# austintheriot/ray-tracer-webgl

Hardware: AMD Instinct MI355X
Metric: Mray/s (ray segments/s) at 1920x1080 (higher is better)
Workload: dtype f32

## Files before the change

profiles/summarize.py:

```python
#!/usr/bin/env python3
import csv
import glob
import json
import os
import sys
from collections import defaultdict

if sys.argv[1] == "--merge":
    dst = os.path.join(os.path.dirname(os.path.abspath(__file__)), "pmc_traffic.json")
    doc = json.load(open(dst)) if os.path.exists(dst) else {}
    recs = doc.get("records") or ([doc] if doc.get("kernel") else [])
    for src in sys.argv[2:]:
        rec = json.load(open(os.path.join(src, "pmc_traffic.json")))
        recs = [r for r in recs if not (r.get("kernel") == rec.get("kernel") and str(r.get("config", "2")) == str(rec.get("config", "2")))]
        recs.append(rec)
        print("merged %s config %s from %s" % (rec.get("kernel"), rec.get("config"), src))
    recs.sort(key=lambda r: str(r.get("config", "2")))
    json.dump({"note": "one record per (kernel, config): the counter-derived figures bench.py attaches (labelled PRIOR) to a line of the "
                       "same kernel, config and launch shape; written by profiles/summarize.py from a profiles/collect.sh run",
               "records": recs}, open(dst, "w"), indent=1)
    sys.exit(0)
d = sys.argv[1]
out = {}
bench = {}
try:
    for line in open(os.path.join(d, "kt.log")):
        if line.startswith("{") and '"metric"' in line:
            bench = json.loads(line)
except Exception:
    bench = {}
cfg_name = (bench.get("config", {}).get("workload", "config2").split(":")[0] or "config2")
cfg_key = cfg_name.replace("config", "")
ppl = int(bench.get("config", {}).get("passes_per_launch", 64))
spp_pass = int(bench.get("config", {}).get("spp_per_pass", 16))
for f in glob.glob(os.path.join(d, "kt", "**", "*_kernel_stats.csv"), recursive=True):
    print("== kernel-trace stats (%s)" % os.path.relpath(f, d))
    for row in csv.DictReader(open(f)):
        if row["Name"].startswith("pt_"):
            print("  %-24s calls %s avg %.3f ms min %.3f max %.3f  (%s %%)" % (
                row["Name"], row["Calls"], float(row["AverageNs"]) / 1e6, float(row["MinNs"]) / 1e6,
                float(row["MaxNs"]) / 1e6, row["Percentage"]))
            out.setdefault("kernel_stats", {})[row["Name"]] = {
                "calls": int(row["Calls"]), "avg_ms": float(row["AverageNs"]) / 1e6}
for f in glob.glob(os.path.join(d, "kt", "**", "*_kernel_trace.csv"), recursive=True):
    rows = [r for r in csv.DictReader(open(f)) if r["Kernel_Name"].startswith("pt_trace")]
    by = defaultdict(list)
    for r in rows:
        by[r["Kernel_Name"]].append((int(r["End_Timestamp"]) - int(r["Start_Timestamp"])) / 1e6)
    print("== full-size dispatches per trace kernel (%s)" % os.path.relpath(f, d))
    for k, v in sorted(by.items()):
        full = [x for x in v if x >= 0.85 * max(v)]
        print("  %-32s %d of %d dispatches full-size: avg %.3f ms  min %.3f  max %.3f" % (k, len(full), len(v), sum(full) / len(full), min(full), max(full)))
        out.setdefault("kernel_full", {})[k] = {"calls": len(full), "avg_ms": sum(full) / len(full)}
for f in glob.glob(os.path.join(d, "kt_configs", "**", "*_kernel_trace.csv"), recursive=True):
    print("== trace-kernel dispatches of tools/config_sweep.py config3 config4 config5 default (%s)" % os.path.relpath(f, d))
    rows = [r for r in csv.DictReader(open(f)) if r["Kernel_Name"].startswith("pt_trace")]
    rows.sort(key=lambda r: int(r["Start_Timestamp"]))
    for r in rows:
        print("  %-32s %9.3f ms  grid %s threads in workgroups of %s  lds %s B  vgpr %s+%s sgpr %s" % (
            r["Kernel_Name"], (int(r["End_Timestamp"]) - int(r["Start_Timestamp"])) / 1e6, r.get("Grid_Size_X", "?"),
            r.get("Workgroup_Size_X", "?"), r.get("LDS_Block_Size", "?"), r.get("VGPR_Count", "?"),
            r.get("Accum_VGPR_Count", "?"), r.get("SGPR_Count", "?")))
for f in glob.glob(os.path.join(d, "kt_configs.log")):
    print("== tools/config_sweep.py output under the profiler")
    for line in open(f):
        if line.startswith(("config", "default")):
            print("  " + line.rstrip())
ctr = defaultdict(lambda: defaultdict(list))
seen_in = defaultdict(set)
for f in sorted(glob.glob(os.path.join(d, "pmc*", "**", "*_counter_collection.csv"), recursive=True)):
    rows = [r for r in csv.DictReader(open(f))]
    pass_dir = os.path.relpath(f, d).split(os.sep)[0]
    longest = defaultdict(float)
    for row in rows:
        dur = float(int(row["End_Timestamp"]) - int(row["Start_Timestamp"]))
        longest[row["Kernel_Name"]] = max(longest[row["Kernel_Name"]], dur)
    for row in rows:
        dur = float(int(row["End_Timestamp"]) - int(row["Start_Timestamp"]))
        if dur >= 0.85 * longest[row["Kernel_Name"]]:
            key = (row["Kernel_Name"], row["Counter_Name"])
            if seen_in[key] and pass_dir not in seen_in[key]:
                continue
            seen_in[key].add(pass_dir)
            ctr[row["Kernel_Name"]][row["Counter_Name"]].append((int(row["Dispatch_Id"]), float(row["Counter_Value"])))
main_kernel = None
if ctr:
    cands = [k for k in ctr if k.startswith("pt_trace")]
    main_kernel = max(cands, key=lambda k: max(len(v) for v in ctr[k].values())) if cands else None
for k in sorted(ctr):
    if not k.startswith("pt_trace"):
        continue
    print("== PMC per dispatch of %s (mean over dispatches; summed over XCDs/SEs by rocprofv3)%s" % (
        k, "  <-- timed kernel" if k == main_kernel else ""))
    vals = {}
    for name in sorted(ctr[k]):
        per = defaultdict(float)
        for disp, v in ctr[k][name]:
            per[disp] += v
        mean = sum(per.values()) / max(len(per), 1)
        vals[name] = mean
        print("  %-28s %.6g" % (name, mean))
    if k == main_kernel:
        out["pmc"] = vals
        out["pmc_kernel"] = k
    g = vals
    if "SQ_INSTS_VALU" in g and "GRBM_GUI_ACTIVE" in g:
        print("  -- derived: cycles per VALU instruction per SIMD = %.3f" % ((g["GRBM_GUI_ACTIVE"] / 8.0) * 1024.0 / g["SQ_INSTS_VALU"]))
    if "FETCH_SIZE" in g:
        print("  FETCH_SIZE KiB %.6g -> bytes %.6g (x2 if wide coalesced: %.6g)" % (g["FETCH_SIZE"], g["FETCH_SIZE"] * 1024, g["FETCH_SIZE"] * 2048))
    if "WRITE_SIZE" in g:
        print("  WRITE_SIZE KiB %.6g -> bytes %.6g" % (g["WRITE_SIZE"], g["WRITE_SIZE"] * 1024))
pm = out.get("pmc", {})
# ... 31 lines not shown
```

ray_tracer_webgl_amd/csrc/pt_api.hip:

```cpp
#include <hip/hip_runtime.h>

#include <mutex>
#include <chrono>
#include <cmath>
#include <cstdarg>
#include <cstdio>
#include <cstdlib>
#include <cstring>
#include <new>
#include <string>
#include <thread>
#include <utility>
#include <vector>

#include "../../include/ptrace.h"
#include "../../include/ptrace_dev.h"
#include "pt_bvh.hpp"
#include "pt_grid.hpp"
#include "pt_grid_records.hpp"
#include "pt_scene_image.hpp"
#include "pt_extra.h"
#include "pt_kernel_args.h"
#include "pt_geom_plan.hpp"
#include "pt_launch_plan.hpp"
// ... 981 lines not shown
    A.lds_scene_bytes = (uint32_t)scene;
  } else {
    const bool have_lds = c->list.n <= PT_MAX_SPHERES_LDS;
    scene = have_lds ? (size_t)PT_LDS_ENTRIES(c->list.n) * 16 : 0;
    row = path == PT_GEOM_SMALL ? ROW_SMALL + (int)(c->list.n & 3u)
                                : (path == PT_GEOM_LDS ? ROW_LIST_LDS : (have_lds ? ROW_SCALAR : ROW_SCALAR_NOLDS));
  }
  const int build = feat ? BUILD_FEAT : (dbg ? BUILD_DBG : (rr ? BUILD_RR : (c->count_work ? BUILD_TWIN : BUILD_PLAIN)));
  if (feat) {
    A.uuid = c->list.uuid.get();
    A.slot_uuid = path == PT_GEOM_BVH ? c->bvh.uuid.get() : (path == PT_GEOM_GRID ? c->grid.uuid.get() : nullptr);
    A.slab = reinterpret_cast<float*>(c->d_feat.get());
    A.spp = 1; A.max_depth = 1; A.rr_min_depth = 0;
  }
  if (walk && path == PT_GEOM_GRID && row == ROW_GRID && (build == BUILD_PLAIN || build == BUILD_TWIN)) {
    A.grid_cells = c->grid.ring.get();
    A.n_cells = (uint32_t)ptrec::ring_cells(c->grid.head.n[0], c->grid.head.n[2]);
  }
  const TraceKernel& tk = kTraceKernels[row][build];
  const void* kfn = tk.main ? tk.main
                            : (tk.feature >= 0 ? feature_kernel(c->device, tk.feature)
                            : tk.debug >= 0 ? debug_kernel(c->device, tk.debug)
                                             : (tk.extra >= 0 ? extra_kernel(c->device, tk.extra) : pt_small_kernel((unsigned)tk.small)));
  c->last_build = build;
  const uint32_t block = walk ? walk_block_threads(kfn, tk.waves, scene, kWalkLdsMax, knobs.bvh_block) : list_block_threads(scene);
  const size_t lds = walk ? scene + (size_t)PT_PARK_STRIDE * 4 * block : scene;
  A.block_threads = block;
  int per_cu = 0;
  PT_HIP(c, resident_blocks(kfn, block, lds, tk.waves, &per_cu));

  const LaunchPlan P = plan_launch({A.n_items, feat ? 1 : c->params.samples_per_pixel, n_passes, block, per_cu, (uint32_t)c->num_cus, walk,
                                    c->list.n, knobs});
  A.queue_chunk = P.queue_chunk; A.queue_static = (uint32_t)P.deal; A.queue_groups = P.queue_groups;
  A.n_waves = P.n_waves; A.coop_max_live = P.coop_max_live;
  A.cost_feedback = use.feedback == LaunchUse::PLANNED ? P.cost_feedback : (use.feedback == LaunchUse::ON ? 1u : 0u);
  if (feat) A.cost_feedback = 0u;
  L->kfn = kfn; L->grid = P.grid; L->block = block; L->lds = lds; L->path = path; L->trial = choice.trial;
  return PT_OK;
}

static int launch_trace(pt_ctx* c, const Launch& L) {
  void* kargs[] = {const_cast<PtKernelArgs*>(&L.A)};
  PT_HIP(c, hipLaunchKernel(L.kfn, dim3(L.grid), dim3(L.block), kargs, L.lds, c->stream));
  return PT_OK;
}

PT_API int pt_render_passes(pt_ctx* c, uint32_t n_passes) {
  if (!c) return PT_ERR_INVALID;
  if (!c->have_spheres || !c->have_params)
    return fail(c, PT_ERR_NOT_READY, "pt_render: pt_set_spheres and pt_set_params must come first");
  if (n_passes == 0) return fail(c, PT_ERR_INVALID, "pt_render_passes: n_passes == 0");
  if (n_passes > c->reserved_passes)
    return fail(c, PT_ERR_CAPACITY, "pt_render_passes: %u passes > %u reserved (pt_reserve_passes)",
                n_passes, c->reserved_passes);
  if (c->local_rows == 0) return PT_OK;
  const bool estimate = c->err_on && !c->err_paused;
  if (estimate && c->err_spp != 0 && c->err_spp != c->params.samples_per_pixel)
    return fail(c, PT_ERR_INVALID, "pt_render_passes: %d samples per pixel while the error estimate holds passes of %d: clear first "
                                   "(pt_reset_accum)", c->params.samples_per_pixel, c->err_spp);
  PT_HIP(c, hipSetDevice(c->device));

  Launch L;
  {
    LaunchUse use;
    use.allow_trials = true;
    int rc = prepare_launch(c, n_passes, use, &L);
    if (rc != PT_OK) return rc;
// ... 978 lines not shown
```

ray_tracer_webgl_amd/csrc/pt_kernel_args.h:

```cpp
#pragma once
#include <stdint.h>

struct PtMatRec {
  float albedo[3];
  float fuzz;
  float refraction_index;
  int32_t type;
  float radius;
  float inv_ri;
};
static_assert(sizeof(PtMatRec) == 32, "PtMatRec must be 32 bytes");
struct PtDiv {
  uint32_t m, s1, s2;
};
static inline PtDiv pt_div_make(uint32_t d) {
  PtDiv r;
  uint32_t l = 0;
  while (l < 32 && (1ull << l) < (unsigned long long)d) l++;
  r.m = (uint32_t)(((1ull << 32) * ((1ull << l) - d)) / d + 1ull);
  r.s1 = l < 1 ? l : 1;
  r.s2 = l > 0 ? l - 1 : 0;
  return r;
}

// ... 25 lines not shown
  const uint32_t* bvh_slot_index;
  const PtMatRec* slot_mat;
  uint32_t n_nodes, n_tree_slots, n_slots, n_outliers;
  float bvh_c0[3], bvh_s0;
  const uint32_t* grid_cells;
  uint32_t n_cells;
  uint32_t grid_n[3];
  float grid_lo[3], grid_hi[3], grid_h[3], grid_inv_h[3];
  float grid_r2_near;
  float grid_lo_n[3], grid_hi_n[3];
  uint32_t lds_scene_bytes;
  unsigned long long* wave_log;
  uint32_t refill_min;
  uint32_t carry_lanes;
  float bvh_kinv;
  uint32_t block_threads;
  uint32_t queue_chunk;
  float fw, fh;
  PtDiv div_per_tile, div_tiles_x, div_band_rows;
  uint32_t coop_max_live;
  int32_t rr_min_depth;
  uint32_t lens_off;
  uint32_t queue_groups;
  uint32_t queue_static;
  uint32_t n_waves;
  uint32_t cost_feedback;
  uint32_t* cell_hist;
  const uint32_t* frame_ctr;
  const float* mat_r0;
  const int32_t* uuid;
  const int32_t* slot_uuid;
  float dbg_cursor[3];
  int32_t dbg_selected;
};

#ifndef PT_WAVES_WALK
#define PT_WAVES_WALK 6
#endif
#ifndef PT_WAVES_LIST
#define PT_WAVES_LIST 7
#endif
#define PT_WAVES_LIST_LDS 6
#ifndef PT_WAVES_SMALL
#define PT_WAVES_SMALL 7
#endif
#define PT_WAVES_TWIN_CELLS 4
#define PT_BUILT_FOR(n) __attribute__((amdgpu_waves_per_eu(n, n)))
#ifndef PT_LEAF_GROUP_GMEM
#define PT_LEAF_GROUP_GMEM 4
#endif

enum { PT_WAVE_LOG_WORDS = 4 };
enum { PT_COH_BINS = 66, PT_HIST_WAVE_STRIDE = 8 };
enum { PT_REG_REFILL_DECODE = 0, PT_REG_REFILL_RESERVE, PT_REG_CAMERA_RAY, PT_REG_SHADE_HIT_RECORD, PT_REG_SHADE_SKY, PT_REG_SHADE_DIFFUSE,
       PT_REG_SHADE_METAL, PT_REG_SHADE_GLASS, PT_REG_SHADE_GLASS_REFRACT, PT_REG_SHADE_CONTINUES, PT_REG_SHADE_FINISHED, PT_REG_SHADE_ITEM_STORE,
       PT_REG_WALK_ENTRY, PT_REG_WALK_ENTER_CELL, PT_REG_WALK_FAR_RAY, PT_REG_SHADE_ANY, PT_N_REGIONS };
enum { PT_CTR_HEAD = 0, PT_CTR_SEGMENTS = 1, PT_CTR_SAMPLES = 2, PT_CTR_FAR_RAYS = 3 , PT_CTR_SCRATCH = 7 , PT_CTR_WORK = 8, PT_CTR_LITERAL = 16, PT_CTR_PHASES = 24, PT_N_PHASES = 8, PT_CTR_REGIONS = 32, PT_CTR_TIMEBINS = 64, PT_CTR_COUNT = 128,
       PT_QUEUE_GROUPS_MAX = 256, PT_CTR_GROUP_HEADS = 128 ,
       PT_CTR_ALLOC = PT_CTR_GROUP_HEADS + 8 * PT_QUEUE_GROUPS_MAX };

#define PT_LDS_ENTRIES(n) ((((n) + 7u) & ~7u) + 4u)
#define PT_MAX_SPHERES_SMALL 16u
#define PT_MAX_SPHERES_LDS 10232u
#define PT_PARK_DWORDS 14u
#ifndef PT_PARK_STRIDE
#define PT_PARK_STRIDE 15u
#endif
#define PT_BVH_LDS_BYTES32(n_nodes, n_slots) ((((size_t)(n_nodes) + 1u) * 2u + (size_t)(n_slots)) * 16u)
#define PT_BVH_LDS_BYTES16(n_nodes) (((size_t)(n_nodes) + 1u) * 16u)
#define PT_GRID_LDS_CELLS(n_cells) ((((size_t)(n_cells) + 3u) / 4u) * 16u)
#define PT_MAX_SPHERES 65528u

enum {
  PT_PROBE_HASH = 0,
  PT_PROBE_SINCOS = 1,
  PT_PROBE_CBRT = 2,
  PT_PROBE_UNIT_SPHERE = 3,
  PT_PROBE_DIVSQRT = 4,
  PT_PROBE_BASE_HASH = 5,
  PT_PROBE_FAST_ARITH = 6,
};
```

ray_tracer_webgl_amd/csrc/pt_launch_plan.hpp:

```cpp
#pragma once
#include <cstdint>
#include <optional>

#include "pt_kernel_args.h"

struct LaunchKnobs {
  std::optional<uint32_t> carry_lanes;
  std::optional<uint32_t> bvh_block;
  std::optional<uint32_t> coop_max;
  std::optional<int> per_cu;
  std::optional<uint32_t> queue_chunk;
  std::optional<uint32_t> grid_percent;
  std::optional<bool> queue_static;
  std::optional<bool> cost_feedback;
  std::optional<int> fewer_x10_1, fewer_x10_2;
  std::optional<bool> queue_grouped;
};

struct LaunchPlanIn {
  uint64_t items = 0;
  int spp = 1;
  uint32_t passes = 1;
  uint32_t block = 256;
  int per_cu = 1;
  uint32_t num_cus = 256;
  bool walk = false;
  uint32_t n_spheres = 0;
  LaunchKnobs knobs;
};

enum class Deal : uint32_t { Shared = 0, Static = 1, Grouped = 2 };

struct LaunchPlan {
  uint32_t queue_chunk = 0;
  Deal deal = Deal::Shared;
  uint32_t queue_groups = 0;
  uint32_t grid = 1;
  uint32_t n_waves = 0;
  uint32_t cost_feedback = 0;
  uint32_t coop_max_live = 0;
};

inline uint32_t list_block_threads(uint64_t lds) { return lds > 40 * 1024 ? 1024u : 256u; }

inline LaunchPlan plan_launch(const LaunchPlanIn& in) {
  const LaunchKnobs& k = in.knobs;
  const uint64_t items = in.items;
  const uint32_t block = in.block;
  LaunchPlan P;
  P.cost_feedback = (in.passes >= 2u || in.spp >= 8) ? 1u : 0u;
  if (!in.walk) {
    const uint32_t per_ray = (in.n_spheres / 64u + 1u) * 60u + 60u;
    const uint32_t lim = (12u * in.n_spheres + 700u) / per_ray;
    P.coop_max_live = lim > 16u ? 16u : lim;
    if (k.coop_max) P.coop_max_live = *k.coop_max;
  }
  int per_cu = in.per_cu < 1 ? 1 : in.per_cu;
  if (k.per_cu && *k.per_cu >= 1 && *k.per_cu <= 32) per_cu = *k.per_cu;

  {
    const unsigned long long lanes = (unsigned long long)in.num_cus * (unsigned)per_cu * block;
    P.queue_chunk = items >= 192ull * lanes ? 512u : (items >= 64ull * lanes ? 128u : (items >= 16ull * lanes ? 64u : 32u));
    {
      const uint32_t spp = (uint32_t)(in.spp > 0 ? in.spp : 1);
      uint32_t c_min = 32u;
      while (c_min * spp < 1100u && c_min < 1024u) c_min *= 2u;
      if (P.queue_chunk < c_min) P.queue_chunk = c_min;
    }
    if (k.queue_chunk && *k.queue_chunk >= 1u && *k.queue_chunk <= 4096u) P.queue_chunk = *k.queue_chunk;
  }
  const unsigned long long want = (items + block - 1) / block;
  const unsigned long long resident = (unsigned long long)in.num_cus * (unsigned)per_cu;
  uint32_t grid = (uint32_t)(want < resident ? want : resident);
  if (k.grid_percent) grid = (uint32_t)((unsigned long long)grid * *k.grid_percent / 100ull);
  if (grid < 1) grid = 1;
  P.grid = grid;
  P.n_waves = grid * (block / 64u);
  const unsigned long long lanes_all = (unsigned long long)P.n_waves * 64ull;
// ... 35 lines not shown
```

ray_tracer_webgl_amd/csrc/pt_refill.hpp:

```cpp
#pragma once
#include "pt_scene.hpp"

namespace ptk {

struct PixelDiv {
  bool wh_ok;
  float y_fw, y_fh;
};
__device__ __forceinline__ PixelDiv pixel_div() {
  karg_t& K = *kargs();
  PixelDiv pd;
  pd.wh_ok = div_den_ok(K.fw) && div_den_ok(K.fh);
  pd.y_fw = u2f((uint32_t)__builtin_amdgcn_readfirstlane((int)f2u(rcp_newton(K.fw))));
  pd.y_fh = u2f((uint32_t)__builtin_amdgcn_readfirstlane((int)f2u(rcp_newton(K.fh))));
  return pd;
}

template <bool FEAT = false>
__device__ __forceinline__ void start_sample(Path& p, const PixelDiv& pd) {
  karg_t& K = *kargs();
  if constexpr (FEAT) {
    const float s = p.st_s, t = p.st_t;
    const V3 dd = mk(fma_(t, K.vertical[0], fma_(s, K.horizontal[0], K.llc[0])),
                     fma_(t, K.vertical[1], fma_(s, K.horizontal[1], K.llc[1])),
// ... 22 lines not shown
  const V3 tt = mk(dd.x - cam_o.x, dd.y - cam_o.y, dd.z - cam_o.z);
  float seed_l = seed;
  seed = (seed + 0.1f) + 0.1f;
  seed = (seed + 0.1f) + 0.1f;
  bool lens = K.lens_off == 0u;
  if (!lens) {
    const uint32_t nz = 0x80000000u;
    lens = pt_ballot(f2u(tt.x) == nz || f2u(tt.y) == nz || f2u(tt.z) == nz) != 0ull;
  }
  if (lens) {
    float ua = hash1(seed_l);
    float sa, ca;
    sincos2pi(ua, sa, ca);
    float rr = sqrt_rn(hash1(seed_l));
    float rdx = K.lens_radius * (rr * ca);
    float rdy = K.lens_radius * (rr * sa);
    V3 off = mk(fma_(K.cam_v[0], rdy, K.cam_u[0] * rdx), fma_(K.cam_v[1], rdy, K.cam_u[1] * rdx),
                fma_(K.cam_v[2], rdy, K.cam_u[2] * rdx));
    d = mk(tt.x - off.x, tt.y - off.y, tt.z - off.z);
    o = mk(cam_o.x + off.x, cam_o.y + off.y, cam_o.z + off.z);
  } else {
    d = tt;
    o = cam_o;
  }
  a = dot3(d, d);
  col = mk(1.0f, 1.0f, 1.0f);
  depth = 0;
  p.seed = seed; p.o = o; p.d = d; p.a = a; p.col = col; p.depth = depth;
}

template <bool COUNT>
__device__ __forceinline__ void refill(const PtKernelArgs& A, Path& p, Queue& q, const PixelDiv& pd, Tally<COUNT>& tally) {
  karg_t& K = *kargs();
  bool alive = p.alive, new_path = p.new_path;
  bool dry = q.dry;
  uint32_t slab_index = p.slab_index, item_tile = p.item_tile, item_segs = p.item_segs;
  int sample = p.sample; float seed = p.seed, st_s = p.st_s, st_t = p.st_t; V3 sum = p.sum;
  uint32_t pool_next = q.pool_next, pool_end = q.pool_end, refill_waited = q.refill_waited;
  uint32_t pool_tp0 = q.pool_tp0, pool_split = q.pool_split, pool_tile0 = q.pool_tile0, pool_tile1 = q.pool_tile1;
  uint32_t q_round = q.round;
  const bool wh_ok = pd.wh_ok;
  const float y_fw = pd.y_fw, y_fh = pd.y_fh;
  bool dealt = false, put_off = false;
  for (;;) {
    bool need = !alive && !dry;
    unsigned long long mask = pt_ballot(need);
    if (mask == 0ull) break;
    if ((uint32_t)__popcll(mask) < K.refill_min && (uint32_t)__popcll(pt_ballot(alive)) >= 32u &&
        (dealt ? 0u : refill_waited) < 8u) {
      put_off = true;
      break;
    }
    dealt = true;
    if (pool_next == pool_end) {
      tally.flag(PT_REG_REFILL_RESERVE);
      unsigned long long base = 0;
      if (K.queue_static == 2u) {
        const uint32_t wave = blockIdx.x * (blockDim.x >> 6) + (threadIdx.x >> 6);
        const uint32_t group = wave & (K.queue_groups - 1u);
        unsigned long long r = 0;
        if (lane_id() == 0u) r = atomicAdd(&A.counters[PT_CTR_GROUP_HEADS + 8u * group], 1ull);
        const uint32_t r_lo = (uint32_t)__builtin_amdgcn_readfirstlane((int)(uint32_t)r);
        base = ((unsigned long long)r_lo * K.queue_groups + group) * (unsigned long long)A.queue_chunk;
      } else if (K.queue_static != 0u) {
        const uint32_t wave = blockIdx.x * (blockDim.x >> 6) + (threadIdx.x >> 6);
        base = ((unsigned long long)q_round * K.n_waves + wave) * (unsigned long long)A.queue_chunk;
        q_round++;
      } else {
        if (lane_id() == 0u) base = atomicAdd(&A.counters[PT_CTR_HEAD], (unsigned long long)A.queue_chunk);
      }
      base = ((unsigned long long)(uint32_t)__builtin_amdgcn_readfirstlane((int)(uint32_t)(base >> 32)) << 32) |
             (unsigned long long)(uint32_t)__builtin_amdgcn_readfirstlane((int)(uint32_t)base);
      if (base >= (unsigned long long)A.n_items) {
        tally.queue_dry();
        dry = true;
        need = false;
      } else {
        pool_next = (uint32_t)base;
        unsigned long long end = base + A.queue_chunk;
        pool_end = end < (unsigned long long)A.n_items ? (uint32_t)end : A.n_items;
        pool_tp0 = div_by(pool_next, K.div_per_tile.m, K.div_per_tile.s1, K.div_per_tile.s2);
        pool_split = (pool_tp0 + 1u) * (64u * K.n_passes);
        const uint32_t n_tiles_w = K.tiles_x * K.tiles_y;
        pool_tile0 = (uint32_t)__builtin_amdgcn_readfirstlane((int)K.tile_order[pool_tp0]);
        pool_tile1 = (uint32_t)__builtin_amdgcn_readfirstlane((int)K.tile_order[pool_tp0 + 1u < n_tiles_w ? pool_tp0 + 1u : pool_tp0]);
      }
    }
    const uint32_t avail = pool_end - pool_next;
    const uint32_t cnt = (uint32_t)__popcll(mask);
    const uint32_t rank = (uint32_t)__popcll(mask & ((1ull << lane_id()) - 1ull));
    const uint32_t pool_base = pool_next;
    pool_next += cnt < avail ? cnt : avail;
    if (need && rank < avail) {
      tally.flag(PT_REG_REFILL_DECODE);
      uint32_t item = pool_base + rank;
      uint32_t per_tile = 64u * K.n_passes;
      uint32_t tile_pos, tile;
      if (K.queue_chunk <= per_tile) {
        const bool second = item >= pool_split;
        tile_pos = pool_tp0 + (second ? 1u : 0u);
        const uint32_t t0 = pool_tile0, t1 = pool_tile1;
        tile = second ? t1 : t0;
      } else {
        tile_pos = div_by(item, K.div_per_tile.m, K.div_per_tile.s1, K.div_per_tile.s2);
        tile = K.tile_order[tile_pos];
      }
      uint32_t rem_i = item - tile_pos * per_tile;
      uint32_t pass = rem_i >> 6, l = rem_i & 63u;
      uint32_t ty = div_by(tile, K.div_tiles_x.m, K.div_tiles_x.s1, K.div_tiles_x.s2), tx = tile - ty * K.tiles_x;
      uint32_t px = tx * 8u + (l & 7u), ly = ty * 8u + (l >> 3);
      if (px < K.width && ly < K.local_rows) {
        uint32_t y = ly;
        if (K.band_count > 1u) {
          uint32_t b = div_by(ly, K.div_band_rows.m, K.div_band_rows.s1, K.div_band_rows.s2), r = ly - b * K.band_rows;
          y = (b * K.band_count + K.band_index) * K.band_rows + r;
        }
        const float fx2 = (float)(2u * px + 1u), fy2 = (float)(2u * y + 1u);
        float vx, vy;
        if (wh_ok) { vx = div_core(fx2, K.fw, y_fw) - 1.0f; vy = div_core(fy2, K.fh, y_fh) - 1.0f; }
        else { vx = fx2 / K.fw - 1.0f; vy = fy2 / K.fh - 1.0f; }
        const uint32_t frame_k = *(const uint32_t __attribute__((address_space(4)))*)K.frame_ctr;
        float u_time = K.time0 + (float)(K.first_pass + pass + frame_k) * K.time_step;
        seed = (float)base_hash(f2u(vx), f2u(vy)) * (1.0f / 4294967296.0f) + u_time;
        st_s = (vx + 1.0f) * 0.5f;
        st_t = (vy + 1.0f) * 0.5f;
        slab_index = (pass * K.local_rows + ly) * K.width + px;
        item_tile = (pass == 0u && K.cost_feedback != 0u) ? tile : 0xffffffffu;
        item_segs = 0;
        sum = mk(0.f, 0.f, 0.f);
        sample = 0;
        new_path = true;
        alive = true;
      }
    }
  }
  refill_waited = (dealt ? 0u : refill_waited) + (put_off ? 1u : 0u);
  p.alive = alive; p.new_path = new_path;
  p.slab_index = slab_index; p.item_tile = item_tile; p.item_segs = item_segs;
  p.sample = sample; p.seed = seed; p.st_s = st_s; p.st_t = st_t; p.sum = sum;
  q.pool_next = pool_next; q.pool_end = pool_end; q.refill_waited = refill_waited;
  q.pool_tp0 = pool_tp0; q.pool_split = pool_split; q.pool_tile0 = pool_tile0; q.pool_tile1 = pool_tile1;
  q.round = q_round; q.dry = dry;
}

}
```

ray_tracer_webgl_amd/csrc/pt_scene.hpp:

```cpp
#pragma once
#include "pt_arith.hpp"
#include "pt_kernel_args.h"

namespace ptk {
using namespace ptd;

extern __shared__ float4 pt_lds[];

typedef float f4v __attribute__((ext_vector_type(4)));
typedef const f4v __attribute__((address_space(4))) const_f4v;
typedef const PtKernelArgs __attribute__((address_space(4))) karg_t;

__device__ __forceinline__ karg_t* kargs() { return (karg_t*)__builtin_amdgcn_kernarg_segment_ptr(); }

__device__ __forceinline__ uint32_t lane_id() { return threadIdx.x & 63u; }

__device__ __forceinline__ uint32_t div_by(uint32_t n, uint32_t m, uint32_t s1, uint32_t s2) {
  const uint32_t t = __umulhi(m, n);
  return (t + ((n - t) >> s1)) >> s2;
}

struct Path {
  bool alive = false;
  bool new_path = false;
  uint32_t slab_index = 0;
  uint32_t item_tile = 0xffffffffu, item_segs = 0;
  int sample = 0, depth = 0;
  float seed = 0.f, st_s = 0.f, st_t = 0.f;
  V3 o = mk(0, 0, 0), d = mk(0, 0, 0);
  float a = 0.f;
  V3 col = mk(1, 1, 1), sum = mk(0, 0, 0);
};

struct Queue {
  uint32_t pool_next = 0, pool_end = 0;
  uint32_t refill_waited = 0;
  uint32_t pool_tp0 = 0, pool_split = 0, pool_tile0 = 0, pool_tile1 = 0;
  uint32_t round = 0;
  bool dry = false;
};

struct Hit {
  float closest = PT_MAX_T;
  int hit = -1;
  uint32_t lit_from = 0xffffffffu;
};

struct Carry {
  bool carried = false;
  float closest_w = PT_MAX_T;
  uint32_t hit_pos = 0xffffffffu;
};
struct BvhWalk {
  uint32_t cur = 0, l0 = 0, l1 = 0, l2 = 0, l3 = 0, l_cnt = 0;
  uint32_t q0 = 0, q1 = 0, q2 = 0, q3 = 0, q_cnt = 0;
};
struct GridWalk {
  float tmx = 0.f, tmy = 0.f, tmz = 0.f, t_exit = 0.f;
  uint32_t cell = 0, rem = 0, pend = 0;
};

template <bool SCAN_LDS_, bool HAVE_LDS_, int WALK_, int TAIL_ = -1, bool FLAT_Y_ = false>
struct Scene {
  static constexpr bool SCAN_LDS = SCAN_LDS_, HAVE_LDS = HAVE_LDS_;
  static constexpr int WALK = WALK_;
  static constexpr bool BVH = WALK >= 1 && WALK <= 3;
  static constexpr bool GRID = WALK >= 4 && WALK <= 6;
  static constexpr bool FLAT_Y = FLAT_Y_;
  static_assert(!FLAT_Y_ || WALK_ == 4, "the one-layer walk exists for the LDS-staged grid build");
// ... 169 lines not shown
  __device__ __forceinline__ void carried(bool c) { if constexpr (COUNT) n_carried += (uint32_t)__popcll(pt_ballot(c)); }
  __device__ __forceinline__ void literal(const PtKernelArgs& A, bool irregular, bool handed_over, uint32_t slab_index) {
    if constexpr (COUNT) {
      const unsigned long long mi = pt_ballot(irregular), mh = pt_ballot(handed_over);
      if ((mi | mh) != 0ull && lane_id() == 0) {
        atomicAdd(&A.counters[PT_CTR_LITERAL + 0], (unsigned long long)__popcll(mi));
        atomicAdd(&A.counters[PT_CTR_LITERAL + 1], (unsigned long long)__popcll(mh));
        atomicAdd(&A.counters[PT_CTR_LITERAL + 2], 1ull);
      }
      if (irregular) A.counters[PT_CTR_LITERAL + 3] = 1ull + slab_index;
      else if (handed_over) A.counters[PT_CTR_LITERAL + 4] = 1ull + slab_index;
    }
  }
  __device__ __forceinline__ void queue_dry() { if constexpr (COUNT) { if (t_wave_dry == 0) t_wave_dry = __builtin_amdgcn_s_memrealtime(); } }
  __device__ __forceinline__ void phase(int k) {
    if constexpr (COUNT) {
      const unsigned long long now_ = __builtin_amdgcn_s_memtime();
      ph_t[k] += now_ - ph_mark;
      ph_mark = now_;
    }
  }
  __device__ __forceinline__ void timebin(const PtKernelArgs& A, bool shade) {
    if constexpr (COUNT) {
      const uint32_t bin = (uint32_t)(__builtin_amdgcn_s_memrealtime() >> 16) & 63u;
      if (bin != tb_bin) {
        if (lane_id() == 0 && tb_acc) atomicAdd(&A.counters[PT_CTR_TIMEBINS + tb_bin], (unsigned long long)tb_acc);
        tb_bin = bin; tb_acc = 0;
      }
      tb_acc += (uint32_t)__popcll(pt_ballot(shade));
    }
  }
  __device__ __forceinline__ void flush(const PtKernelArgs& A) {
    if constexpr (COUNT) {
      if (lane_id() < 2u * PT_N_REGIONS && reg_acc != 0u) atomicAdd(&A.counters[PT_CTR_REGIONS + lane_id()], (unsigned long long)reg_acc);
      if (lane_id() == 0) {
        atomicAdd(&A.counters[PT_CTR_WORK + 0], (unsigned long long)n_walk_it);
        atomicAdd(&A.counters[PT_CTR_WORK + 1], (unsigned long long)n_walk_ln);
        atomicAdd(&A.counters[PT_CTR_WORK + 2], (unsigned long long)n_leaf_it);
        atomicAdd(&A.counters[PT_CTR_WORK + 3], (unsigned long long)n_leaf_ln);
        atomicAdd(&A.counters[PT_CTR_WORK + 4], (unsigned long long)n_exact_it);
        atomicAdd(&A.counters[PT_CTR_WORK + 5], (unsigned long long)n_exact_ln);
        atomicAdd(&A.counters[PT_CTR_WORK + 6], (unsigned long long)n_steps);
        atomicAdd(&A.counters[PT_CTR_WORK + 7], (unsigned long long)n_carried);
        atomicAdd(&A.counters[PT_CTR_LITERAL + 5], (unsigned long long)n_exact_always_it);
        atomicAdd(&A.counters[PT_CTR_LITERAL + 6], (unsigned long long)n_exact_always_ln);
        atomicAdd(&A.counters[PT_CTR_LITERAL + 7], (unsigned long long)n_walk_first);
        if (tb_acc) atomicAdd(&A.counters[PT_CTR_TIMEBINS + tb_bin], (unsigned long long)tb_acc);
        for (int k = 0; k < PT_N_PHASES; k++) atomicAdd(&A.counters[PT_CTR_PHASES + k], ph_t[k]);

        if (A.wave_log) {
          unsigned long long* wl = A.wave_log + (unsigned long long)PT_WAVE_LOG_WORDS * (blockIdx.x * (blockDim.x >> 6) + (threadIdx.x >> 6));
          wl[0] = t_wave_start; wl[1] = t_wave_dry; wl[2] = __builtin_amdgcn_s_memrealtime();
          wl[3] = (unsigned long long)hw_id | ((unsigned long long)xcc_id << 32);
        }
      }
    }
  }
};

__device__ __forceinline__ uint32_t first_candidate(uint32_t mask) {
  return (uint32_t)__builtin_ctz(mask | 16u);
}

template <typename G>
__device__ __forceinline__ void sphere_test(const V3& o, const V3& d, float a, const G& g, float& half_b, float& c, float& disc) {
  V3 oc = mk(o.x - g.x, o.y - g.y, o.z - g.z);
  half_b = dot3(oc, d);
// ... 6 lines not shown
```

ray_tracer_webgl_amd/csrc/pt_trace_body.hpp:

```cpp
#pragma once
#include <hip/hip_runtime.h>
#include <stdint.h>

#include "pt_kernel_args.h"
#include "pt_arith.hpp"
#include "pt_scene.hpp"
#include "pt_refill.hpp"
#include "pt_list.hpp"
#include "pt_bvh_walk.hpp"
#include "pt_grid_walk.hpp"
#include "pt_shade.hpp"

using namespace ptd;

template <bool SCAN_LDS, bool HAVE_LDS, int WALK = 0, bool COUNT = false, bool RR = false, int TAIL = -1, bool FLAT_Y = false, bool DBG = false, bool FEAT = false>
__device__ __forceinline__ void pt_trace_body(const PtKernelArgs& A) {
  using namespace ptk;
  using S = Scene<SCAN_LDS, HAVE_LDS, WALK, TAIL, FLAT_Y>;
  S::stage(A);

  Path p;
  Queue q;
  Carry cw;
  BvhWalk bw;
  GridWalk gw;
  Tally<COUNT> tally;
  const PixelDiv pd = pixel_div();
  uint32_t seg_count = 0;
  tally.start();

  for (;;) {
    refill<COUNT>(A, p, q, pd, tally);
    tally.phase(0);
    if (p.alive && p.new_path) {
      tally.flag(PT_REG_CAMERA_RAY);
      start_sample<FEAT>(p, pd);
      p.new_path = false;
    }
    tally.phase(1);
    const unsigned long long live = pt_ballot(p.alive);
    if (live == 0ull) break;
    tally.step();

    Hit h;
    if constexpr (S::TREE) h.closest = cw.carried ? cw.closest_w : PT_MAX_T;
    if (!cw.carried) cw.hit_pos = 0xffffffffu;
    const bool fast = regular_ray(A, p);
    const int n_live = (int)__popcll(live);
    if constexpr (S::TREE) park_store(A, p);
    constexpr bool kTail = !S::TREE && !S::SMALL;
    const bool coop = kTail && (n_live <= (int)A.coop_max_live) && (pt_ballot(p.alive && !fast) == 0ull) &&
                      (pt_ballot(cw.carried) == 0ull);
    if (coop) {
      tail_mode<S>(A, p, live, h);
    } else {
      h.lit_from = fast ? 0xffffffffu : 0u;
      const bool scan_lane = p.alive && fast;
      if constexpr (S::BVH) bvh_walk<S, COUNT>(A, p, scan_lane, n_live, cw, bw, h, tally);
      else if constexpr (S::GRID) grid_walk<S, COUNT>(A, p, scan_lane, n_live, cw, gw, h, tally);
      else if constexpr (S::SMALL) small_scan<S>(A, p, scan_lane, h);
      else list_scan<S>(A, p, scan_lane, h);
      tally.literal(A, p.alive && !fast, scan_lane && h.lit_from < A.n_spheres, p.slab_index);
      if constexpr (S::GRID && S::WALK != 4) {
        const bool handed_over = scan_lane && h.lit_from == 0u;
        const unsigned long long m_h = pt_ballot(handed_over);
// ... 26 lines not shown
```

Before: 58180.

## Prefetch next work item into a per-lane slot and promote when path ends

```diff
diff --git a/profiles/summarize.py b/profiles/summarize.py
--- a/profiles/summarize.py
+++ b/profiles/summarize.py
@@ -5,6 +5,12 @@
 import os
 import sys
 from collections import defaultdict
+
+def full_size_floor(durations):
+    longest = max(durations)
+    long_ones = sorted(x for x in durations if x >= 0.5 * longest)
+    return 0.85 * long_ones[len(long_ones) // 2]
+
 
 if sys.argv[1] == "--merge":
     dst = os.path.join(os.path.dirname(os.path.abspath(__file__)), "pmc_traffic.json")
@@ -49,7 +55,7 @@
         by[r["Kernel_Name"]].append((int(r["End_Timestamp"]) - int(r["Start_Timestamp"])) / 1e6)
     print("== full-size dispatches per trace kernel (%s)" % os.path.relpath(f, d))
     for k, v in sorted(by.items()):
-        full = [x for x in v if x >= 0.85 * max(v)]
+        full = [x for x in v if x >= full_size_floor(v)]
         print("  %-32s %d of %d dispatches full-size: avg %.3f ms  min %.3f  max %.3f" % (k, len(full), len(v), sum(full) / len(full), min(full), max(full)))
         out.setdefault("kernel_full", {})[k] = {"calls": len(full), "avg_ms": sum(full) / len(full)}
 for f in glob.glob(os.path.join(d, "kt_configs", "**", "*_kernel_trace.csv"), recursive=True):
@@ -71,13 +77,16 @@
 for f in sorted(glob.glob(os.path.join(d, "pmc*", "**", "*_counter_collection.csv"), recursive=True)):
     rows = [r for r in csv.DictReader(open(f))]
     pass_dir = os.path.relpath(f, d).split(os.sep)[0]
-    longest = defaultdict(float)
+    durations = defaultdict(list)
+    for row in rows:
+        durations[(row["Kernel_Name"], row["Dispatch_Id"])] = [float(int(row["End_Timestamp"]) - int(row["Start_Timestamp"]))]
+    per_kernel = defaultdict(list)
+    for (kname, _), dur in durations.items():
+        per_kernel[kname] += dur
+    floor = {kname: full_size_floor(v) for kname, v in per_kernel.items()}
     for row in rows:
         dur = float(int(row["End_Timestamp"]) - int(row["Start_Timestamp"]))
-        longest[row["Kernel_Name"]] = max(longest[row["Kernel_Name"]], dur)
-    for row in rows:
-        dur = float(int(row["End_Timestamp"]) - int(row["Start_Timestamp"]))
-        if dur >= 0.85 * longest[row["Kernel_Name"]]:
+        if dur >= floor[row["Kernel_Name"]]:
             key = (row["Kernel_Name"], row["Counter_Name"])
             if seen_in[key] and pass_dir not in seen_in[key]:
                 continue
diff --git a/ray_tracer_webgl_amd/csrc/pt_api.hip b/ray_tracer_webgl_amd/csrc/pt_api.hip
--- a/ray_tracer_webgl_amd/csrc/pt_api.hip
+++ b/ray_tracer_webgl_amd/csrc/pt_api.hip
@@ -1037,7 +1037,7 @@
   const LaunchPlan P = plan_launch({A.n_items, feat ? 1 : c->params.samples_per_pixel, n_passes, block, per_cu, (uint32_t)c->num_cus, walk,
                                     c->list.n, knobs});
   A.queue_chunk = P.queue_chunk; A.queue_static = (uint32_t)P.deal; A.queue_groups = P.queue_groups;
-  A.n_waves = P.n_waves; A.coop_max_live = P.coop_max_live;
+  A.n_waves = P.n_waves; A.coop_max_live = P.coop_max_live; A.refill_ahead = P.refill_ahead;
   A.cost_feedback = use.feedback == LaunchUse::PLANNED ? P.cost_feedback : (use.feedback == LaunchUse::ON ? 1u : 0u);
   if (feat) A.cost_feedback = 0u;
   L->kfn = kfn; L->grid = P.grid; L->block = block; L->lds = lds; L->path = path; L->trial = choice.trial;
diff --git a/ray_tracer_webgl_amd/csrc/pt_deal.hpp b/ray_tracer_webgl_amd/csrc/pt_deal.hpp
--- /dev/null
+++ b/ray_tracer_webgl_amd/csrc/pt_deal.hpp
@@ -0,0 +1,49 @@
+#pragma once
+#include <stdint.h>
+
+#if defined(__HIPCC__) || defined(__CUDACC__)
+#define PT_DEAL_FN __host__ __device__ __forceinline__
+#else
+#define PT_DEAL_FN inline
+#endif
+
+namespace ptdeal {
+
+constexpr uint32_t kSlotEmpty = 0xffffffffu;
+enum { kQueueShared = 0, kQueueStatic = 1, kQueueGrouped = 2 };
+
+PT_DEAL_FN bool wants_item(bool alive, bool slot_empty, bool dry, bool ahead) { return slot_empty && !dry && (ahead || !alive); }
+PT_DEAL_FN bool starving(bool alive, bool slot_empty, bool dry) { return !alive && slot_empty && !dry; }
+PT_DEAL_FN bool promotes(bool alive, bool slot_empty) { return !alive && !slot_empty; }
+
+PT_DEAL_FN uint32_t popcount64(unsigned long long m) { return (uint32_t)__builtin_popcountll(m); }
+PT_DEAL_FN uint32_t rank_of(unsigned long long mask, uint32_t lane) {
+#if defined(__HIP_DEVICE_COMPILE__)
+  (void)lane;
+  return __builtin_amdgcn_mbcnt_hi((uint32_t)(mask >> 32), __builtin_amdgcn_mbcnt_lo((uint32_t)mask, 0u));
+#else
+  return popcount64(mask & ((1ull << lane) - 1ull));
+#endif
+}
+PT_DEAL_FN uint32_t taken(unsigned long long mask, uint32_t avail) {
+  const uint32_t cnt = popcount64(mask);
+  return cnt < avail ? cnt : avail;
+}
+PT_DEAL_FN bool gets_item(bool need, uint32_t rank, uint32_t avail) { return need && rank < avail; }
+PT_DEAL_FN uint32_t item_of(uint32_t pool_base, uint32_t rank) { return pool_base + rank; }
+
+PT_DEAL_FN bool pool_used_up(uint32_t pool_next, uint32_t pool_end) { return pool_next == pool_end; }
+PT_DEAL_FN unsigned long long grouped_base(uint32_t r, uint32_t groups, uint32_t group, uint32_t chunk) {
+  return ((unsigned long long)r * groups + group) * (unsigned long long)chunk;
+}
+PT_DEAL_FN uint32_t group_of(uint32_t wave, uint32_t groups) { return wave & (groups - 1u); }
+PT_DEAL_FN unsigned long long static_base(uint32_t round, uint32_t n_waves, uint32_t wave, uint32_t chunk) {
+  return ((unsigned long long)round * n_waves + wave) * (unsigned long long)chunk;
+}
+PT_DEAL_FN bool reservation_dry(unsigned long long base, uint32_t n_items) { return base >= (unsigned long long)n_items; }
+PT_DEAL_FN uint32_t reservation_end(unsigned long long base, uint32_t chunk, uint32_t n_items) {
+  const unsigned long long end = base + chunk;
+  return end < (unsigned long long)n_items ? (uint32_t)end : n_items;
+}
+
+}
diff --git a/ray_tracer_webgl_amd/csrc/pt_kernel_args.h b/ray_tracer_webgl_amd/csrc/pt_kernel_args.h
--- a/ray_tracer_webgl_amd/csrc/pt_kernel_args.h
+++ b/ray_tracer_webgl_amd/csrc/pt_kernel_args.h
@@ -81,6 +81,7 @@
   const int32_t* slot_uuid;
   float dbg_cursor[3];
   int32_t dbg_selected;
+  uint32_t refill_ahead;
 };
 
 #ifndef PT_WAVES_WALK
@@ -103,8 +104,9 @@
 enum { PT_COH_BINS = 66, PT_HIST_WAVE_STRIDE = 8 };
 enum { PT_REG_REFILL_DECODE = 0, PT_REG_REFILL_RESERVE, PT_REG_CAMERA_RAY, PT_REG_SHADE_HIT_RECORD, PT_REG_SHADE_SKY, PT_REG_SHADE_DIFFUSE,
        PT_REG_SHADE_METAL, PT_REG_SHADE_GLASS, PT_REG_SHADE_GLASS_REFRACT, PT_REG_SHADE_CONTINUES, PT_REG_SHADE_FINISHED, PT_REG_SHADE_ITEM_STORE,
-       PT_REG_WALK_ENTRY, PT_REG_WALK_ENTER_CELL, PT_REG_WALK_FAR_RAY, PT_REG_SHADE_ANY, PT_N_REGIONS };
-enum { PT_CTR_HEAD = 0, PT_CTR_SEGMENTS = 1, PT_CTR_SAMPLES = 2, PT_CTR_FAR_RAYS = 3 , PT_CTR_SCRATCH = 7 , PT_CTR_WORK = 8, PT_CTR_LITERAL = 16, PT_CTR_PHASES = 24, PT_N_PHASES = 8, PT_CTR_REGIONS = 32, PT_CTR_TIMEBINS = 64, PT_CTR_COUNT = 128,
+       PT_REG_WALK_ENTRY, PT_REG_WALK_ENTER_CELL, PT_REG_WALK_FAR_RAY, PT_REG_SHADE_ANY,
+       PT_REG_REFILL_PROMOTE , PT_N_REGIONS };
+enum { PT_CTR_HEAD = 0, PT_CTR_SEGMENTS = 1, PT_CTR_SAMPLES = 2, PT_CTR_FAR_RAYS = 3 , PT_CTR_REGIONS_MORE = 4 , PT_CTR_SCRATCH = 7 , PT_CTR_WORK = 8, PT_CTR_LITERAL = 16, PT_CTR_PHASES = 24, PT_N_PHASES = 8, PT_CTR_REGIONS = 32, PT_CTR_TIMEBINS = 64, PT_CTR_COUNT = 128,
        PT_QUEUE_GROUPS_MAX = 256, PT_CTR_GROUP_HEADS = 128 ,
        PT_CTR_ALLOC = PT_CTR_GROUP_HEADS + 8 * PT_QUEUE_GROUPS_MAX };
 
diff --git a/ray_tracer_webgl_amd/csrc/pt_launch_plan.hpp b/ray_tracer_webgl_amd/csrc/pt_launch_plan.hpp
--- a/ray_tracer_webgl_amd/csrc/pt_launch_plan.hpp
+++ b/ray_tracer_webgl_amd/csrc/pt_launch_plan.hpp
@@ -39,11 +39,24 @@
   uint32_t n_waves = 0;
   uint32_t cost_feedback = 0;
   uint32_t coop_max_live = 0;
+  uint32_t refill_ahead = 1;
 };
 
 inline uint32_t list_block_threads(uint64_t lds) { return lds > 40 * 1024 ? 1024u : 256u; }
 
+inline uint32_t refill_ahead(uint64_t items, int spp, uint32_t n_waves) {
+  const unsigned long long lanes = (unsigned long long)n_waves * 64ull;
+  return (spp < 32 || 2ull * items >= (unsigned long long)spp * lanes) ? 1u : 0u;
+}
+
+inline LaunchPlan plan_queue(const LaunchPlanIn& in);
 inline LaunchPlan plan_launch(const LaunchPlanIn& in) {
+  LaunchPlan P = plan_queue(in);
+  P.refill_ahead = refill_ahead(in.items, in.spp, P.n_waves);
+  return P;
+}
+
+inline LaunchPlan plan_queue(const LaunchPlanIn& in) {
   const LaunchKnobs& k = in.knobs;
   const uint64_t items = in.items;
   const uint32_t block = in.block;
diff --git a/ray_tracer_webgl_amd/csrc/pt_refill.hpp b/ray_tracer_webgl_amd/csrc/pt_refill.hpp
--- a/ray_tracer_webgl_amd/csrc/pt_refill.hpp
+++ b/ray_tracer_webgl_amd/csrc/pt_refill.hpp
@@ -78,53 +78,46 @@
 template <bool COUNT>
 __device__ __forceinline__ void refill(const PtKernelArgs& A, Path& p, Queue& q, const PixelDiv& pd, Tally<COUNT>& tally) {
   karg_t& K = *kargs();
-  bool alive = p.alive, new_path = p.new_path;
+  const bool alive = p.alive;
   bool dry = q.dry;
-  uint32_t slab_index = p.slab_index, item_tile = p.item_tile, item_segs = p.item_segs;
-  int sample = p.sample; float seed = p.seed, st_s = p.st_s, st_t = p.st_t; V3 sum = p.sum;
-  uint32_t pool_next = q.pool_next, pool_end = q.pool_end, refill_waited = q.refill_waited;
+  uint32_t nx_slab = p.nx_slab, nx_tile = p.nx_tile;
+  float nx_seed = p.nx_seed, nx_s = p.nx_s, nx_t = p.nx_t;
+  uint32_t pool_next = q.pool_next, pool_end = q.pool_end;
   uint32_t pool_tp0 = q.pool_tp0, pool_split = q.pool_split, pool_tile0 = q.pool_tile0, pool_tile1 = q.pool_tile1;
   uint32_t q_round = q.round;
   const bool wh_ok = pd.wh_ok;
   const float y_fw = pd.y_fw, y_fh = pd.y_fh;
-  bool dealt = false, put_off = false;
   for (;;) {
-    bool need = !alive && !dry;
-    unsigned long long mask = pt_ballot(need);
-    if (mask == 0ull) break;
-    if ((uint32_t)__popcll(mask) < K.refill_min && (uint32_t)__popcll(pt_ballot(alive)) >= 32u &&
-        (dealt ? 0u : refill_waited) < 8u) {
-      put_off = true;
-      break;
-    }
-    dealt = true;
-    if (pool_next == pool_end) {
+    const bool slot_empty = nx_slab == ptdeal::kSlotEmpty;
+    if (pt_ballot(ptdeal::starving(alive, slot_empty, dry)) == 0ull) break;
+    bool need = ptdeal::wants_item(alive, slot_empty, dry, K.refill_ahead != 0u);
+    const unsigned long long mask = pt_ballot(need);
+    if (ptdeal::pool_used_up(pool_next, pool_end)) {
       tally.flag(PT_REG_REFILL_RESERVE);
       unsigned long long base = 0;
       if (K.queue_static == 2u) {
         const uint32_t wave = blockIdx.x * (blockDim.x >> 6) + (threadIdx.x >> 6);
-        const uint32_t group = wave & (K.queue_groups - 1u);
+        const uint32_t group = ptdeal::group_of(wave, K.queue_groups);
         unsigned long long r = 0;
         if (lane_id() == 0u) r = atomicAdd(&A.counters[PT_CTR_GROUP_HEADS + 8u * group], 1ull);
         const uint32_t r_lo = (uint32_t)__builtin_amdgcn_readfirstlane((int)(uint32_t)r);
-        base = ((unsigned long long)r_lo * K.queue_groups + group) * (unsigned long long)A.queue_chunk;
+        base = ptdeal::grouped_base(r_lo, K.queue_groups, group, A.queue_chunk);
       } else if (K.queue_static != 0u) {
         const uint32_t wave = blockIdx.x * (blockDim.x >> 6) + (threadIdx.x >> 6);
-        base = ((unsigned long long)q_round * K.n_waves + wave) * (unsigned long long)A.queue_chunk;
+        base = ptdeal::static_base(q_round, K.n_waves, wave, A.queue_chunk);
         q_round++;
       } else {
         if (lane_id() == 0u) base = atomicAdd(&A.counters[PT_CTR_HEAD], (unsigned long long)A.queue_chunk);
       }
       base = ((unsigned long long)(uint32_t)__builtin_amdgcn_readfirstlane((int)(uint32_t)(base >> 32)) << 32) |
              (unsigned long long)(uint32_t)__builtin_amdgcn_readfirstlane((int)(uint32_t)base);
-      if (base >= (unsigned long long)A.n_items) {
+      if (ptdeal::reservation_dry(base, A.n_items)) {
         tally.queue_dry();
         dry = true;
         need = false;
       } else {
         pool_next = (uint32_t)base;
-        unsigned long long end = base + A.queue_chunk;
-        pool_end = end < (unsigned long long)A.n_items ? (uint32_t)end : A.n_items;
+        pool_end = ptdeal::reservation_end(base, A.queue_chunk, A.n_items);
         pool_tp0 = div_by(pool_next, K.div_per_tile.m, K.div_per_tile.s1, K.div_per_tile.s2);
         pool_split = (pool_tp0 + 1u) * (64u * K.n_passes);
         const uint32_t n_tiles_w = K.tiles_x * K.tiles_y;
@@ -133,13 +126,12 @@
       }
     }
     const uint32_t avail = pool_end - pool_next;
-    const uint32_t cnt = (uint32_t)__popcll(mask);
-    const uint32_t rank = (uint32_t)__popcll(mask & ((1ull << lane_id()) - 1ull));
+    const uint32_t rank = ptdeal::rank_of(mask, lane_id());
     const uint32_t pool_base = pool_next;
-    pool_next += cnt < avail ? cnt : avail;
-    if (need && rank < avail) {
+    pool_next += ptdeal::taken(mask, avail);
+    if (ptdeal::gets_item(need, rank, avail)) {
       tally.flag(PT_REG_REFILL_DECODE);
-      uint32_t item = pool_base + rank;
+      uint32_t item = ptdeal::item_of(pool_base, rank);
       uint32_t per_tile = 64u * K.n_passes;
       uint32_t tile_pos, tile;
       if (K.queue_chunk <= per_tile) {
@@ -167,26 +159,32 @@
         else { vx = fx2 / K.fw - 1.0f; vy = fy2 / K.fh - 1.0f; }
         const uint32_t frame_k = *(const uint32_t __attribute__((address_space(4)))*)K.frame_ctr;
         float u_time = K.time0 + (float)(K.first_pass + pass + frame_k) * K.time_step;
-        seed = (float)base_hash(f2u(vx), f2u(vy)) * (1.0f / 4294967296.0f) + u_time;
-        st_s = (vx + 1.0f) * 0.5f;
-        st_t = (vy + 1.0f) * 0.5f;
-        slab_index = (pass * K.local_rows + ly) * K.width + px;
-        item_tile = (pass == 0u && K.cost_feedback != 0u) ? tile : 0xffffffffu;
-        item_segs = 0;
-        sum = mk(0.f, 0.f, 0.f);
-        sample = 0;
-        new_path = true;
-        alive = true;
+        nx_seed = (float)base_hash(f2u(vx), f2u(vy)) * (1.0f / 4294967296.0f) + u_time;
+        nx_s = (vx + 1.0f) * 0.5f;
+        nx_t = (vy + 1.0f) * 0.5f;
+        nx_slab = (pass * K.local_rows + ly) * K.width + px;
+        nx_tile = (pass == 0u && K.cost_feedback != 0u) ? tile : 0xffffffffu;
       }
     }
   }
-  refill_waited = (dealt ? 0u : refill_waited) + (put_off ? 1u : 0u);
-  p.alive = alive; p.new_path = new_path;
-  p.slab_index = slab_index; p.item_tile = item_tile; p.item_segs = item_segs;
-  p.sample = sample; p.seed = seed; p.st_s = st_s; p.st_t = st_t; p.sum = sum;
-  q.pool_next = pool_next; q.pool_end = pool_end; q.refill_waited = refill_waited;
+  p.nx_slab = nx_slab; p.nx_tile = nx_tile; p.nx_seed = nx_seed; p.nx_s = nx_s; p.nx_t = nx_t;
+  q.pool_next = pool_next; q.pool_end = pool_end;
   q.pool_tp0 = pool_tp0; q.pool_split = pool_split; q.pool_tile0 = pool_tile0; q.pool_tile1 = pool_tile1;
   q.round = q_round; q.dry = dry;
 }
 
+template <bool COUNT>
+__device__ __forceinline__ void promote(Path& p, Tally<COUNT>& tally) {
+  if (ptdeal::promotes(p.alive, p.nx_slab == ptdeal::kSlotEmpty)) {
+    tally.flag(PT_REG_REFILL_PROMOTE);
+    p.seed = p.nx_seed; p.st_s = p.nx_s; p.st_t = p.nx_t;
+    p.slab_index = p.nx_slab; p.item_tile = p.nx_tile; p.item_segs = 0;
+    p.sum = mk(0.f, 0.f, 0.f);
+    p.sample = 0;
+    p.new_path = true;
+    p.alive = true;
+    p.nx_slab = ptdeal::kSlotEmpty;
+  }
 }
+
+}
diff --git a/ray_tracer_webgl_amd/csrc/pt_scene.hpp b/ray_tracer_webgl_amd/csrc/pt_scene.hpp
--- a/ray_tracer_webgl_amd/csrc/pt_scene.hpp
+++ b/ray_tracer_webgl_amd/csrc/pt_scene.hpp
@@ -1,5 +1,6 @@
 #pragma once
 #include "pt_arith.hpp"
+#include "pt_deal.hpp"
 #include "pt_kernel_args.h"
 
 namespace ptk {
@@ -30,11 +31,12 @@
   V3 o = mk(0, 0, 0), d = mk(0, 0, 0);
   float a = 0.f;
   V3 col = mk(1, 1, 1), sum = mk(0, 0, 0);
+  uint32_t nx_slab = ptdeal::kSlotEmpty, nx_tile = 0xffffffffu;
+  float nx_seed = 0.f, nx_s = 0.f, nx_t = 0.f;
 };
 
 struct Queue {
   uint32_t pool_next = 0, pool_end = 0;
-  uint32_t refill_waited = 0;
   uint32_t pool_tp0 = 0, pool_split = 0, pool_tile0 = 0, pool_tile1 = 0;
   uint32_t round = 0;
   bool dry = false;
@@ -270,7 +272,8 @@
   }
   __device__ __forceinline__ void flush(const PtKernelArgs& A) {
     if constexpr (COUNT) {
-      if (lane_id() < 2u * PT_N_REGIONS && reg_acc != 0u) atomicAdd(&A.counters[PT_CTR_REGIONS + lane_id()], (unsigned long long)reg_acc);
+      if (lane_id() < 2u * PT_N_REGIONS && reg_acc != 0u)
+        atomicAdd(&A.counters[lane_id() < 32u ? PT_CTR_REGIONS + lane_id() : PT_CTR_REGIONS_MORE + (lane_id() - 32u)], (unsigned long long)reg_acc);
       if (lane_id() == 0) {
         atomicAdd(&A.counters[PT_CTR_WORK + 0], (unsigned long long)n_walk_it);
         atomicAdd(&A.counters[PT_CTR_WORK + 1], (unsigned long long)n_walk_ln);
diff --git a/ray_tracer_webgl_amd/csrc/pt_trace_body.hpp b/ray_tracer_webgl_amd/csrc/pt_trace_body.hpp
--- a/ray_tracer_webgl_amd/csrc/pt_trace_body.hpp
+++ b/ray_tracer_webgl_amd/csrc/pt_trace_body.hpp
@@ -31,6 +31,7 @@
 
   for (;;) {
     refill<COUNT>(A, p, q, pd, tally);
+    promote<COUNT>(p, tally);
     tally.phase(0);
     if (p.alive && p.new_path) {
       tally.flag(PT_REG_CAMERA_RAY);
```

After: 61150, median of 6. +5.1%, better.
